# LYL232/Experiment-Distributed-Deep-Learning

Hardware: AMD Instinct MI355X
Metric: device-resident allreduce GiB/s vs bucket size at 1/2/4/8 MI355X (higher is better)
Workload: dtype f32; 1 GPU; C2: local reduce kernel acc += in (per-hop ring reduce), fp32, 256 MiB bucket, 1xMI355X; bucket_bytes=268435456, parallelism=none (1 GPU)

## Files before the change

experiment-distributed-deep-learning_amd/csrc/c_api.cpp:

```cpp
#include <algorithm>
#include <cstdlib>
#include <cstring>
#include <map>
#include <memory>
#include <string>
#include <tuple>
#include <vector>

#include "engine.h"
#include "abi.h"
#include "handler.h"

using namespace ddl;
using namespace ddl::abi;

namespace {

std::shared_ptr<ReadyEvent> ready_event(int memory, void *hip_stream) {
    DDL_REQUIRE(memory == DDL_MEMORY_DEVICE || memory == DDL_MEMORY_HOST, DDL_STATUS_INVALID_ARGUMENT,
                "memory must be DDL_MEMORY_DEVICE (0) or DDL_MEMORY_HOST (1), not " << memory);
    return memory == DDL_MEMORY_HOST ? nullptr : std::make_shared<ReadyEvent>(as_stream(hip_stream));
}

}

extern "C" {

int ddl_version(void) { return 2; }

#ifndef DDL_SRC_HASH
#define DDL_SRC_HASH "unknown"
#endif
const char *ddl_build_info(void) { return "src=" DDL_SRC_HASH " arch=gfx950"; }
const char *ddl_last_error(void) { return last_error(); }
const char *ddl_dtype_name(int dtype) { return dtype_name(dtype); }
size_t ddl_dtype_size(int dtype) { return dtype_size(dtype); }

int ddl_get_unique_id(void *out, size_t len) {
    return guarded([&] {
        DDL_REQUIRE(out && len >= sizeof(ncclUniqueId), DDL_STATUS_INVALID_ARGUMENT,
                    "unique id buffer needs " << sizeof(ncclUniqueId) << " bytes");
        ncclUniqueId id;
        rccl_check(rccl().GetUniqueId(&id), "ncclGetUniqueId");
        std::memcpy(out, &id, sizeof id);
    });
}

int ddl_init(int rank, int size, int device, const void *unique_id, size_t len) {
    return guarded([&] {
        DDL_REQUIRE(size >= 1 && rank >= 0 && rank < size, DDL_STATUS_INVALID_ARGUMENT,
                    "bad rank/size " << rank << "/" << size);
        DDL_REQUIRE(!Registry::get().initialized(), DDL_STATUS_INVALID_ARGUMENT, "already initialized");
        DDL_HIP(hipSetDevice(device));
        ncclComm_t nc = size > 1 ? rccl_init_rank(rank, size, unique_id, len) : nullptr;
        Registry::get().set_world(new_communicator(rank, size, device, nc));
        DDL_LOG(1, "initialized rank " << rank << "/" << size << " on device " << device
                                       << (size > 1 ? std::string(" rccl=") + rccl().path : ""));
    });
}

int ddl_init_single(int device) { return ddl_init(0, 1, device, nullptr, 0); }

int ddl_control_listen(char *endpoint_out, size_t len) {
    return guarded([&] {
        std::string ep = standalone_control()->listen();
        DDL_REQUIRE(endpoint_out && len > ep.size(), DDL_STATUS_INVALID_ARGUMENT, "endpoint buffer too small");
        std::memcpy(endpoint_out, ep.c_str(), ep.size() + 1);
    });
}

int ddl_control_connect(const char *endpoints) {
    return guarded([&] {
        DDL_REQUIRE(endpoints, DDL_STATUS_INVALID_ARGUMENT, "null endpoints");
        auto world = Registry::get().world();
        auto ch = standalone_control();
        ch->connect(world->rank(), world->size(), split_endpoints(endpoints), 120000);
        standalone_control() = std::make_shared<ControlChannel>();
        world->enable_keyed(ch);
    });
}

int ddl_control_stats(long long *string_rounds, long long *cached_rounds) {
    return guarded([&] {
        DDL_REQUIRE(string_rounds && cached_rounds, DDL_STATUS_INVALID_ARGUMENT, "null output");
        ControlChannel *ch = standalone_control().get();
        if (Registry::get().initialized() && Registry::get().world()->control())
            ch = Registry::get().world()->control();
        *string_rounds = ch->string_rounds;
        *cached_rounds = ch->cached_rounds;
    });
}

int ddl_finalize(void) {
    return guarded([&] {
        Registry::get().clear();
        DDL_REQUIRE(wait_deferred_deletions(60000), DDL_STATUS_ERROR_UNKNOWN,
                    "a communicator released by its own handler thread is still being destroyed after 60 s");
        free_retired();
        standalone_control() = std::make_shared<ControlChannel>();
        run_finalize_hooks();
    });
}

int ddl_is_initialized(void) { return Registry::get().initialized() ? 1 : 0; }

int ddl_set_config(const char *key, long long value) {
    return guarded([&] {
        DDL_REQUIRE(key, DDL_STATUS_INVALID_ARGUMENT, "null key");
        std::string k(key);
        Config &c = config();
        if (k == "slice_bytes") c.slice_bytes = value;
        else if (k == "algo") {
            DDL_REQUIRE(value >= kAlgoRing && value <= kAlgoDirectGather, DDL_STATUS_INVALID_ARGUMENT,
                        "algo must be 0 (ring), 1 (direct), 2 (one-shot), 3 (gather-fold) or 4 (direct-gather)");
            c.algo = value;
        } else if (k == "rings") c.rings = value;
        else if (k == "max_slices") c.max_slices = value;
        else if (k == "fusion_threshold_bytes") {
            DDL_REQUIRE(value > 0, DDL_STATUS_INVALID_ARGUMENT, "fusion threshold must be > 0");
            c.fusion_threshold_bytes = value;
        } else if (k == "log_level") c.log_level = value;
        else if (k == "cycle_time_us") c.cycle_time_us = value;
        else if (k == "host_chunk_bytes") {
            DDL_REQUIRE(value >= 4096, DDL_STATUS_INVALID_ARGUMENT, "host_chunk_bytes must be >= 4096");
            c.host_chunk_bytes = value;
        } else if (k == "host_copy_threads") {
            DDL_REQUIRE(value >= 0 && value <= 64, DDL_STATUS_INVALID_ARGUMENT, "host_copy_threads must be in [0, 64]");
            c.host_copy_threads = value;
        } else if (k == "host_zero_copy") c.host_zero_copy = value ? 1 : 0;
        else if (k == "host_numa_bind") c.host_numa_bind = value ? 1 : 0;
        else if (k == "host_register_cache_bytes") {
            DDL_REQUIRE(value >= 0, DDL_STATUS_INVALID_ARGUMENT, "host_register_cache_bytes must be >= 0");
            c.host_register_cache_bytes = value;
            if (value == 0)
                for (auto &comm : Registry::get().all())
                    if (RequestHandler *h = comm->handler_if_created()) h->release_registrations();
        }
        else if (k == "tune") c.tune = value ? 1 : 0;
        else if (k == "fusion_pipeline_bytes") {
            DDL_REQUIRE(value >= 0, DDL_STATUS_INVALID_ARGUMENT, "fusion_pipeline_bytes must be >= 0");
            c.fusion_pipeline_bytes = value;
        } else if (k == "one_rank_shortcut") c.one_rank_shortcut = value ? 1 : 0;
        else if (k == "pipeline_rounds") c.pipeline_rounds = value ? 1 : 0;
        else if (k == "reference_order") c.reference_order = value ? 1 : 0;
        else if (k == "capture_mode") {
            DDL_REQUIRE(value != 1, DDL_STATUS_INVALID_ARGUMENT,
                        "capture_mode 1 (forked streams) was removed in r04: HIP 7.0's hipStreamEndCapture crashes "
                        "on three or more cross-waiting forked streams (DESIGN §9); 2 keeps the overlap");
            DDL_REQUIRE(value == 0 || value == 2, DDL_STATUS_INVALID_ARGUMENT,
                        "capture_mode must be 0 (serial) or 2 (single-stream DAG)");
            c.capture_mode = value;
        } else if (k == "compute_cu_mask") {
            DDL_REQUIRE(value == 0 || value == 2 || value == 4 || value == 8, DDL_STATUS_INVALID_ARGUMENT,
                        "compute_cu_mask must be 0 (all CUs), 2, 4 or 8 (every n-th CU left to RCCL)");
            c.compute_cu_mask = value;
        } else if (k == "queue_isolation") c.queue_isolation = value ? 1 : 0;
        else if (k == "rccl_min_ctas" || k == "rccl_max_ctas") {
            DDL_REQUIRE(value >= 0 && value <= 256, DDL_STATUS_INVALID_ARGUMENT,
                        k << " must be 0 (RCCL's default) or a channel count in [1, 256]");
            (k == "rccl_min_ctas" ? c.rccl_min_ctas : c.rccl_max_ctas) = value;
        } else if (k == "fold_form") {
            DDL_REQUIRE(value >= 0 && value <= 2, DDL_STATUS_INVALID_ARGUMENT,
                        "fold_form must be 0 (auto), 1 (tile form) or 2 (run form)");
            set_fold_form((int)value);
        }
        else fail(DDL_STATUS_INVALID_ARGUMENT, "unknown config key '" + k + "'");
        c.epoch.fetch_add(1);
    });
}

long long ddl_get_config(const char *key) {
    if (!key) return -1;
    std::string k(key);
    Config &c = config();
    if (k == "slice_bytes") return c.slice_bytes;
    if (k == "algo") return c.algo;
    if (k == "rings") return c.rings;
    if (k == "max_slices") return c.max_slices;
    if (k == "fusion_threshold_bytes") return c.fusion_threshold_bytes;
    if (k == "log_level") return c.log_level;
    if (k == "cycle_time_us") return c.cycle_time_us;
    if (k == "host_chunk_bytes") return c.host_chunk_bytes;
    if (k == "tune") return c.tune;
    if (k == "host_copy_threads") return c.host_copy_threads;
    if (k == "host_zero_copy") return c.host_zero_copy;
    if (k == "host_register_cache_bytes") return c.host_register_cache_bytes;
    if (k == "host_numa_bind") return c.host_numa_bind;
    if (k == "host_registered_bytes") return c.host_registered_bytes;
    if (k == "host_register_failures") return c.host_register_failures;
    if (k == "host_register_hits") return c.host_register_hits;
    if (k == "host_unregistered_ranges") return c.host_unregistered_ranges;
    if (k == "host_zero_copy_plans") return c.host_zero_copy_plans;
    if (k == "host_pack_us") return c.host_pack_ns / 1000;
    if (k == "host_wait_us") return c.host_wait_ns / 1000;
    if (k == "host_unpack_us") return c.host_unpack_ns / 1000;
    if (k == "host_check_us") return c.host_check_ns / 1000;
    if (k == "host_plan_us") return c.host_plan_ns / 1000;
    if (k == "host_coll_us") return c.host_coll_ns / 1000;
    if (k == "host_d2h_post_us") return c.host_d2h_post_ns / 1000;
    if (k == "host_unpack_submit_us") return c.host_unpack_submit_ns / 1000;
    if (k == "host_lane_d2h_wait_us") return c.host_lane_d2h_wait_ns / 1000;
    if (k == "host_lane_copy_us") return c.host_lane_copy_ns / 1000;
    if (k == "host_lane_copy_bytes") return c.host_lane_copy_bytes;
    if (k == "host_lane_jobs") return c.host_lane_jobs;
    if (k == "fusion_pipeline_bytes") return c.fusion_pipeline_bytes;
    if (k == "one_rank_shortcut") return c.one_rank_shortcut;
    if (k == "pipeline_rounds") return c.pipeline_rounds;
    if (k == "reference_order") return c.reference_order;
    if (k == "capture_mode") return c.capture_mode;
    if (k == "fold_form") return get_fold_form();
    if (k == "compute_cu_mask") return c.compute_cu_mask;
    if (k == "queue_isolation") return c.queue_isolation;
    if (k == "rccl_min_ctas") return c.rccl_min_ctas;
    if (k == "rccl_max_ctas") return c.rccl_max_ctas;
    return -1;
}

int communicator_rank(ddl_communicator_id id) {
    int r = -1;
    if (guarded([&] { r = Registry::get().find(id)->rank(); }) != DDL_STATUS_OK) return -1;
    return r;
}

int communicator_size(ddl_communicator_id id) {
    int s = -1;
    if (guarded([&] { s = Registry::get().find(id)->size(); }) != DDL_STATUS_OK) return -1;
    return s;
}

ddl_communicator_id world_communicator(void) {
    ddl_communicator_id id = 0;
    if (guarded([&] { id = Registry::get().world()->id(); }) != DDL_STATUS_OK) return 0;
    return id;
}

ddl_communicator_id split_communicator(ddl_communicator_id id, int color, int key) {
    ddl_communicator_id out = 0;
    int st = guarded([&] {
        auto c = Registry::get().find(id)->split(color, key);
        Registry::get().add(c);
        out = c->id();
    });
    return st == DDL_STATUS_OK ? out : 0;
}

void detach_communicator(ddl_communicator_id id) {
    (void)guarded([&] { Registry::get().detach(id); });
}

void py_info(const char *s) { DDL_LOG(1, "[py]: " << (s ? s : "")); }
void py_debug(const char *s) { DDL_LOG(2, "[py]: " << (s ? s : "")); }
void py_error(const char *s) { DDL_LOG(0, "[py]: " << (s ? s : "")); }

int ddl_allreduce(ddl_communicator_id id, const void *send, void *recv, size_t elements, int dtype,
                  int op, void *hip_stream) {
    return guarded([&] { Registry::get().find(id)->allreduce(send, recv, elements, dtype, op, as_stream(hip_stream)); });
}

int ddl_allreduce_batch(ddl_communicator_id id, int count, const void *const *sends, void *const *recvs,
                        const size_t *elements, int dtype, int op, void *hip_stream) {
    return guarded([&] {
        Registry::get().find(id)->allreduce_batch(sends, recvs, elements, count, dtype, op, as_stream(hip_stream));
    });
}

int ddl_broadcast(ddl_communicator_id id, void *buf, size_t elements, int dtype, int root, void *hip_stream) {
    return guarded([&] { Registry::get().find(id)->broadcast(buf, elements, dtype, root, as_stream(hip_stream)); });
}

int ddl_allgatherv(ddl_communicator_id id, const void *send, size_t send_elements, void *recv,
                   const size_t *recv_counts, const size_t *displs, int dtype, void *hip_stream) {
    return guarded([&] {
        auto c = Registry::get().find(id);
        DDL_REQUIRE(recv_counts && displs, DDL_STATUS_INVALID_ARGUMENT, "null counts/displs");
        DDL_REQUIRE(recv_counts[c->rank()] == send_elements, DDL_STATUS_INVALID_ARGUMENT,
                    "send_elements " << send_elements << " != recv_counts[rank] " << recv_counts[c->rank()]);
        c->allgatherv(send, recv, recv_counts, displs, dtype, as_stream(hip_stream));
    });
}

int ddl_allgather(ddl_communicator_id id, const void *send, size_t send_elements, void *recv, size_t recv_elements,
                  int dtype, void *hip_stream) {
    return guarded([&] {
        auto c = Registry::get().find(id);
        DDL_REQUIRE(send_elements == recv_elements, DDL_STATUS_INVALID_ARGUMENT,
                    "send_elements " << send_elements << " != recv_elements " << recv_elements);
        std::vector<size_t> counts(c->size(), recv_elements), displs(c->size());
        for (int q = 0; q < c->size(); ++q) displs[q] = (size_t)q * recv_elements;
        c->allgatherv(send, recv, counts.data(), displs.data(), dtype, as_stream(hip_stream));
    });
}

int ddl_allreduce_host(ddl_communicator_id id, const void *send, void *recv, size_t elements, int dtype, int op) {
    return guarded([&] { Registry::get().find(id)->allreduce_host(send, recv, elements, dtype, op); });
}

int ddl_comm_transport(ddl_communicator_id id, int *kind, int *ranks) {
    return guarded([&] {
        DDL_REQUIRE(kind && ranks, DDL_STATUS_INVALID_ARGUMENT, "null output");
        Registry::get().find(id)->transport(kind, ranks);
    });
}

int ddl_tune_result(ddl_communicator_id id, size_t bucket_bytes, int *chosen, int *count, long long *configs,
                    float *ms, int max_candidates) {
    return guarded([&] {
        export_tune(Registry::get().find(id)->tune_result(bucket_bytes), chosen, count, configs, ms, max_candidates);
    });
}

int ddl_allreduce_submit_mem(ddl_communicator_id id, const char *key, const void *in, void *out, size_t elements,
                             int dtype, int op, int memory, void *hip_stream, ddl_done_fn done, void *user) {
    return guarded([&] {
        DDL_REQUIRE(key, DDL_STATUS_INVALID_ARGUMENT, "null key");
        auto c = Registry::get().find(id);
        DeviceGuard g(c->device());
        Request r;
        r.key = key;
        r.in = in;
        r.out = out;
        r.n = elements;
        r.dtype = dtype;
        r.op = op;
        r.done = done;
        r.user = user;
        r.host = memory == DDL_MEMORY_HOST;
        r.ready = ready_event(memory, hip_stream);
        c->handler().submit(r);
    });
}

int ddl_allreduce_submit(ddl_communicator_id id, const char *key, const void *in, void *out, size_t elements,
                         int dtype, int op, void *hip_stream, ddl_done_fn done, void *user) {
    return ddl_allreduce_submit_mem(id, key, in, out, elements, dtype, op, DDL_MEMORY_DEVICE, hip_stream, done, user);
}

int ddl_broadcast_submit_mem(ddl_communicator_id id, const char *key, const void *in, void *out, size_t elements,
                             int dtype, int root, int memory, void *hip_stream, ddl_done_fn done, void *user) {
    return guarded([&] {
        DDL_REQUIRE(key, DDL_STATUS_INVALID_ARGUMENT, "null key");
        auto c = Registry::get().find(id);
        DeviceGuard g(c->device());
        Request r;
        r.type = kReqBroadcast;
        r.key = key;
        r.in = in;
        r.out = out;
        r.n = elements;
        r.dtype = dtype;
        r.root = root;
        r.done = done;
        r.user = user;
        r.host = memory == DDL_MEMORY_HOST;
        r.ready = ready_event(memory, hip_stream);
        c->handler().submit(r);
    });
}

int ddl_broadcast_submit(ddl_communicator_id id, const char *key, const void *in, void *out, size_t elements,
                         int dtype, int root, void *hip_stream, ddl_done_fn done, void *user) {
    return ddl_broadcast_submit_mem(id, key, in, out, elements, dtype, root, DDL_MEMORY_DEVICE, hip_stream, done,
                                    user);
}

int ddl_allgather_submit_mem(ddl_communicator_id id, const char *key, const void *in, size_t first_dim,
                             size_t row_elements, int dtype, int memory, void *hip_stream, ddl_alloc_fn alloc,
                             ddl_done_fn done, void *user) {
    return guarded([&] {
        DDL_REQUIRE(key, DDL_STATUS_INVALID_ARGUMENT, "null key");
        auto c = Registry::get().find(id);
        DeviceGuard g(c->device());
        Request r;
        r.type = kReqAllgather;
        r.key = key;
        r.in = in;
        r.first_dim = first_dim;
        r.row_elems = row_elements;
        r.n = first_dim * row_elements;
        r.dtype = dtype;
        r.alloc = alloc;
        r.done = done;
        r.user = user;
        r.host = memory == DDL_MEMORY_HOST;
        r.ready = ready_event(memory, hip_stream);
        c->handler().submit(r);
    });
}

int ddl_allgather_submit(ddl_communicator_id id, const char *key, const void *in, size_t first_dim, size_t row_elements,
                         int dtype, void *hip_stream, ddl_alloc_fn alloc, ddl_done_fn done, void *user) {
    return ddl_allgather_submit_mem(id, key, in, first_dim, row_elements, dtype, DDL_MEMORY_DEVICE, hip_stream, alloc,
                                    done, user);
}

int ddl_allreduce_submit_batch_mem(ddl_communicator_id id, int count, const char *const *keys, const void *const *ins,
                                   void *const *outs, const size_t *elements, const int *dtypes, int op, int memory,
                                   void *hip_stream, ddl_done_fn done, void *const *users) {
    return guarded([&] {
        DDL_REQUIRE(count >= 0 && (count == 0 || (keys && ins && outs && elements && dtypes)),
                    DDL_STATUS_INVALID_ARGUMENT, "bad batch arguments");
        if (count == 0) return;
        auto c = Registry::get().find(id);
        DeviceGuard g(c->device());
        auto ready = ready_event(memory, hip_stream);
        std::vector<Request> rs(count);
        for (int i = 0; i < count; ++i) {
            DDL_REQUIRE(keys[i], DDL_STATUS_INVALID_ARGUMENT, "null key " << i);
            rs[i].key = keys[i];
            rs[i].in = ins[i];
            rs[i].out = outs[i];
            rs[i].n = elements[i];
            rs[i].dtype = dtypes[i];
            rs[i].op = op;
            rs[i].done = done;
            rs[i].user = users ? users[i] : nullptr;
            rs[i].host = memory == DDL_MEMORY_HOST;
            rs[i].ready = ready;
        }
        c->handler().submit_batch(rs);
    });
}

int ddl_allreduce_submit_batch(ddl_communicator_id id, int count, const char *const *keys, const void *const *ins,
                               void *const *outs, const size_t *elements, const int *dtypes, int op,
                               void *hip_stream, ddl_done_fn done, void *const *users) {
    return ddl_allreduce_submit_batch_mem(id, count, keys, ins, outs, elements, dtypes, op, DDL_MEMORY_DEVICE,
                                          hip_stream, done, users);
}

int ddl_kernel_timing(ddl_communicator_id id, int on) {
    return guarded([&] {
        auto c = Registry::get().find(id);
        std::lock_guard<std::mutex> g(c->mutex());
        c->executor().set_timing(on != 0);
    });
}

int ddl_kernel_stats(ddl_communicator_id id, long long *launches, double *bytes, double *ms) {
    return guarded([&] {
        DDL_REQUIRE(launches && bytes && ms, DDL_STATUS_INVALID_ARGUMENT, "null output");
        auto c = Registry::get().find(id);
        std::lock_guard<std::mutex> g(c->mutex());
        DeviceGuard dg(c->device());
        KernelStats s = c->executor().collect_stats();
        *launches = s.launches;
        *bytes = s.bytes;
        *ms = s.ms;
    });
}

int ddl_host_unregister(const void *ptr, size_t bytes) {
    return guarded([&] {
        for (auto &comm : Registry::get().all())
            if (RequestHandler *h = comm->handler_if_created()) h->unregister_range(ptr, bytes);
    });
}

int ddl_wait_all(ddl_communicator_id id) {
    return guarded([&] { Registry::get().find(id)->handler().wait_all(); });
}

}
```

experiment-distributed-deep-learning_amd/csrc/common.h:

```cpp
#pragma once

#include <hip/hip_runtime.h>

#include <algorithm>
#include <cstddef>
#include <cstdint>
#include <cstdio>
#include <string>
#include <sstream>
#include <vector>

#include "ddl_amd_testing.h"

namespace ddl {

inline size_t dtype_size(int dt) {
    switch (dt) {
        case DDL_FLOAT: case DDL_INT32: return 4;
        case DDL_DOUBLE: case DDL_INT64: case DDL_UINT64: return 8;
        case DDL_HALF: case DDL_BFLOAT16: return 2;
        default: return 0;
    }
}

inline const char *dtype_name(int dt) {
    switch (dt) {
        case DDL_FLOAT: return "float32";
        case DDL_DOUBLE: return "float64";
        case DDL_INT32: return "int32";
        case DDL_INT64: return "int64";
        case DDL_UINT64: return "uint64";
        case DDL_HALF: return "float16";
        case DDL_BFLOAT16: return "bfloat16";
        default: return "unsupported";
    }
}

void set_error(const std::string &msg);
const char *last_error();

struct Error {
    int status;
    std::string msg;
};

[[noreturn]] inline void fail(int status, const std::string &msg) { throw Error{status, msg}; }

#define DDL_HIP(expr)                                                                       \
    do {                                                                                    \
        hipError_t _e = (expr);                                                             \
        if (_e != hipSuccess) {                                                             \
            std::ostringstream _os;                                                         \
            _os << #expr << " failed: " << hipGetErrorString(_e) << " (" << __FILE__ << ":" \
                << __LINE__ << ")";                                                         \
            ::ddl::fail(DDL_STATUS_HIP_ERROR, _os.str());                                   \
        }                                                                                   \
    } while (0)

#define DDL_REQUIRE(cond, status, msg)                    \
    do {                                                  \
        if (!(cond)) {                                    \
            std::ostringstream _os;                       \
            _os << msg;                                   \
            ::ddl::fail((status), _os.str());             \
        }                                                 \
    } while (0)

int log_level();
void log_line(int level, const std::string &msg);

#define DDL_LOG(level, msg)                                     \
    do {                                                        \
        if (::ddl::log_level() >= (level)) {                    \
            std::ostringstream _os;                             \
            _os << msg;                                         \
            ::ddl::log_line((level), _os.str());                \
        }                                                       \
    } while (0)

#define DDL_TRACE(msg)                                                                          \
    do {                                                                                        \
        if (::ddl::log_level() >= 4) {                                                          \
            std::ostringstream _os;                                                             \
            _os << msg;                                                                         \
            std::fprintf(stderr, "[ddl trace] %s\n", _os.str().c_str());                         \
            std::fflush(stderr);                                                                \
        }                                                                                       \
    } while (0)

constexpr int kMaxSegments = 8;

struct SegTable {
    const void *a[kMaxSegments];
    const void *b[kMaxSegments];
    void *out[kMaxSegments];
    uint64_t n[kMaxSegments];
    int count;
};

constexpr int kMaxInputs = 15;
enum FoldOrder : int {
    kFoldLeft = 0,
    kFoldMpichTree = 1,
    kFoldBinomial = 2,
};
inline int mpich_fold_order(size_t message_bytes, size_t esize, int P) {
    size_t pof2 = 1;
    while (pof2 * 2 <= (size_t)P) pof2 *= 2;
    return message_bytes <= 2048 || message_bytes / esize < pof2 ? kFoldBinomial : kFoldMpichTree;
}
struct SegTableN {
    const void *a;
    const void *b[kMaxInputs];
    void *out;
    uint64_t n;
    int nb;
    int order = kFoldLeft;
};
void launch_sumN(const SegTableN &t, int dtype, hipStream_t stream);
constexpr int kMaxFoldBatch = 8;
struct FoldBatch {
    SegTableN t[kMaxFoldBatch];
    int count;
};
void launch_sumN_batch(const SegTableN *t, int count, int dtype, hipStream_t stream);

enum ReduceVariant : int {
    kNtLoadA = 1,
    kNtLoadB = 2,
    kNtStore = 4,
    kLdsStageB = 8,
    kWtStore = 16,
    kVariantMask = 31,
    kRunForm = 32,
    kRun4 = 64,
};
int default_variant(size_t bytes);
int ring_variant();
void set_fold_form(int form);
void set_testing_fold_variant(int v);
int get_fold_form();

void launch_sum2(const SegTable &t, int dtype, hipStream_t stream, int variant = -1);
int device_cu_count();

inline std::vector<size_t> host_chunk_cuts(size_t total, size_t chunk) {
    std::vector<size_t> cut{0};
    while (cut.back() < total) cut.push_back(cut.back() + std::min(chunk, total - cut.back()));
    return cut;
}

class SegmentCopier {
public:
    SegmentCopier() = default;
    ~SegmentCopier();
    SegmentCopier(const SegmentCopier &) = delete;
    SegmentCopier &operator=(const SegmentCopier &) = delete;
    void run(int dir, void *flat, void *const *segs, const size_t *bytes, int count, hipStream_t stream);
    static size_t flat_bytes(const size_t *bytes, int count);

private:
    struct Slot {
        void *host = nullptr, *dev = nullptr;
        size_t cap = 0;
        void *idx = nullptr;
        size_t idx_cap = 0;
        hipEvent_t ready = nullptr;
    };
    Slot &free_slot_();
    static constexpr size_t kMaxSlots = 64;
    std::vector<Slot> slots_;
    size_t next_ = 0;
};

void retire_device(void *p);
void retire_host(void *p);
void free_retired();
void *thread_scratch(size_t bytes);

enum class QueueClass { kPooled, kHigh, kLow };

}
```

experiment-distributed-deep-learning_amd/csrc/engine.h:

```cpp
#pragma once

#include <atomic>
#include <condition_variable>
#include <functional>
#include <map>
#include <memory>
#include <mutex>
#include <string>
#include <utility>
#include <vector>

#include "control.h"
#include "executor.h"

namespace ddl {

class RequestHandler;

struct Config {
    std::atomic<long long> algo{kAlgoRing};
    std::atomic<long long> slice_bytes{2ll << 20};
    std::atomic<long long> rings{kMaxRings};
    std::atomic<long long> max_slices{8};
    std::atomic<long long> fusion_threshold_bytes{(1ll << 31) - 1};
    std::atomic<long long> log_level{0};
    std::atomic<long long> cycle_time_us{0};
    std::atomic<long long> host_chunk_bytes{32ll << 20};
    std::atomic<long long> host_copy_threads{7};
    std::atomic<long long> host_zero_copy{1};
    std::atomic<long long> host_register_cache_bytes{0};
    std::atomic<long long> host_numa_bind{1};
    std::atomic<long long> host_registered_bytes{0};
    std::atomic<long long> host_register_failures{0};
    std::atomic<long long> host_register_hits{0};
    std::atomic<long long> host_unregistered_ranges{0};
    std::atomic<long long> host_zero_copy_plans{0};
    std::atomic<long long> host_pack_ns{0};
    std::atomic<long long> host_wait_ns{0};
    std::atomic<long long> host_unpack_ns{0};
    std::atomic<long long> host_check_ns{0};
    std::atomic<long long> host_plan_ns{0};
    std::atomic<long long> host_coll_ns{0};
    std::atomic<long long> host_d2h_post_ns{0};
    std::atomic<long long> host_unpack_submit_ns{0};
    std::atomic<long long> host_lane_d2h_wait_ns{0};
    std::atomic<long long> host_lane_copy_ns{0};
    std::atomic<long long> host_lane_copy_bytes{0};
    std::atomic<long long> host_lane_jobs{0};
    std::atomic<long long> tune{1};
    std::atomic<long long> fusion_pipeline_bytes{256ll << 20};
    std::atomic<long long> one_rank_shortcut{1};
    std::atomic<long long> pipeline_rounds{1};
    std::atomic<long long> reference_order{1};
    std::atomic<long long> capture_mode{0};
    std::atomic<long long> compute_cu_mask{0};
    std::atomic<long long> rccl_min_ctas{0};
    std::atomic<long long> rccl_max_ctas{0};
    std::atomic<long long> queue_isolation{0};
    std::atomic<long long> epoch{0};
    uint64_t shared_hash() const;
    RingConfig ring() const {
        RingConfig c;
        c.algo = (int)algo.load();
        c.rings = (int)rings.load();
        c.slice_bytes = (size_t)slice_bytes.load();
        c.max_slices = (int)max_slices.load();
        c.ref_order = reference_order.load() ? 1 : 0;
        return c;
    }
};
Config &config();

struct TuneResult {
    std::vector<RingConfig> candidates;
    std::vector<float> ms;
    int chosen = -1;
};

int size_class(size_t bytes);

TuneResult run_tuning(int P, size_t bytes, hipStream_t stream, const RingConfig &base,
                      const std::function<void(const RingConfig &)> &run,
                      const std::function<void(float *, int)> &agree_max);

class Communicator {
public:
    Communicator(int rank, int size, int device, ncclComm_t nccl, std::shared_ptr<TestHooks> hooks = nullptr,
                 long long tag = 0, std::vector<int> world_ranks = {}, QueueClass qc = QueueClass::kPooled);
    ~Communicator();

    long long id() const { return reinterpret_cast<long long>(this); }
    int rank() const { return rank_; }
    int size() const { return size_; }
    int device() const { return device_; }
    QueueClass queue_class() const { return qclass_; }
    QueueClass keyed_queue_class() const { return keyed_qclass_; }
    ncclComm_t nccl() const { return nccl_; }

    void allreduce(const void *send, void *recv, size_t n, int dtype, int op, hipStream_t stream,
                   size_t order_bytes = 0);
    void allreduce_batch(const void *const *send, void *const *recv, const size_t *n, int count, int dtype, int op,
                         hipStream_t stream);
    void allreduce_host(const void *send, void *recv, size_t n, int dtype, int op);
    void broadcast(void *buf, size_t n, int dtype, int root, hipStream_t stream);
    void allgatherv(const void *send, void *recv, const size_t *counts, const size_t *displs, int dtype,
                    hipStream_t stream);
    std::shared_ptr<Communicator> split(int color, int key, bool keyed = true);

    RingConfig ring_config(size_t n, int dtype, hipStream_t stream);
    TuneResult tune_result(size_t bytes);

    RequestHandler &handler();
    RequestHandler *handler_if_created();
    ControlChannel *control() const { return control_.get(); }
    void enable_keyed(std::shared_ptr<ControlChannel> ch);
    std::shared_ptr<Communicator> keyed_data() const { return keyed_data_; }
    RingExecutor &executor() { return *exec_; }
    std::mutex &mutex() { return mu_; }
    void rccl_allreduce(const void *send, void *recv, size_t n, int dtype, hipStream_t stream);
    void transport(int *kind, int *ranks) const;

    long long round_freeze();
    void round_release(long long at);
    void round_enter(long long at);
    void round_unfreeze();
    void round_abort(int status, const std::string &why);
    long long user_collectives() const;
    std::vector<long long> round_log() const;

    void agree_config(hipStream_t stream);

private:
    class UserCollective;
    std::mutex gate_mu_;
    std::condition_variable gate_cv_;
    long long user_seq_ = 0;
    long long user_done_ = 0;
    bool frozen_ = false;
    int aborted_ = 0;
    std::string abort_msg_;
    long long release_ = 0;
    std::vector<long long> round_log_;
    uint64_t agreed_hash_ = 0;
    uint64_t tuned_hash_ = 0;
    hipStream_t ctl_stream_ = nullptr;
    void agree_max_(float *values, int count, hipStream_t stream);

    int rank_, size_, device_;
    ncclComm_t nccl_;
    std::shared_ptr<TestHooks> hooks_;
    long long tag_ = 0;
    std::vector<int> world_ranks_;
    Transport *cb_ = nullptr;
    std::mutex mu_;
    std::unique_ptr<RingExecutor> exec_;
    std::shared_ptr<ControlChannel> control_;
    std::shared_ptr<Communicator> keyed_data_;
    std::unique_ptr<RequestHandler> handler_;
    std::mutex handler_mu_;
    std::map<int, TuneResult> tuned_;
    TuneResult tune_(size_t n, int dtype, hipStream_t stream, const RingConfig &base);
    hipStream_t h2d_ = nullptr, ring_ = nullptr, d2h_ = nullptr;
    static constexpr int kHostSlots = 4;
    void *slots_[kHostSlots] = {};
    size_t slot_bytes_ = 0;
    void *tune_a_ = nullptr, *tune_b_ = nullptr;
    size_t tune_cap_ = 0;
    QueueClass qclass_ = QueueClass::kPooled, keyed_qclass_ = QueueClass::kPooled;
};

extern thread_local bool t_handler_thread;

struct CommunicatorDeleter {
    void operator()(Communicator *c) const;
};
bool wait_deferred_deletions(long long limit_ms);


template <class... A>
std::shared_ptr<Communicator> new_communicator(A &&...a) {
    return std::shared_ptr<Communicator>(new Communicator(std::forward<A>(a)...), CommunicatorDeleter{});
}

class Registry {
public:
    static Registry &get();
    void add(const std::shared_ptr<Communicator> &c);
    std::shared_ptr<Communicator> find(long long id);
    void detach(long long id);
    std::shared_ptr<Communicator> world();
    std::vector<std::shared_ptr<Communicator>> all();
    void set_world(const std::shared_ptr<Communicator> &c);
    void clear();
    bool initialized();

private:
    std::mutex mu_;
    std::map<long long, std::shared_ptr<Communicator>> comms_;
    std::shared_ptr<Communicator> world_;
};

void add_finalize_hook(void (*fn)());
void run_finalize_hooks();

class DeviceGuard {
public:
    explicit DeviceGuard(int device);
    ~DeviceGuard();

private:
    int prev_ = -1;
};

ncclComm_t rccl_init_rank(int rank, int size, const void *unique_id, size_t len);
ncclComm_t rccl_split(ncclComm_t parent, int color, int key, int *rank, int *size);
void rccl_max_floats(ncclComm_t comm, float *values, int count, hipStream_t stream);
void rccl_allgather_u64(ncclComm_t comm, uint64_t *values, int size, int rank, hipStream_t stream);
void check_config_agreement(int rank, const std::vector<uint64_t> &hashes);

}
```

experiment-distributed-deep-learning_amd/csrc/pack.hip:

```cpp
#include <hip/hip_runtime.h>

#include <algorithm>
#include <cstdlib>
#include <cstring>
#include <mutex>
#include <vector>

#include "common.h"
#include "deptrace.h"

namespace ddl {

namespace {

using u32x4 = unsigned int __attribute__((ext_vector_type(4)));

struct SegDesc {
    uint64_t ptr;
    uint64_t off;
    uint64_t len;
    uint32_t vec;
    uint32_t tile0;
};

__device__ inline void copy_bytes(char *dst, const char *src, uint32_t m) {
    for (uint32_t k = 0; k < m; ++k) dst[k] = src[k];
}

constexpr uint32_t kIdxBlock = 128;

template <bool NARROW>
__global__ void __launch_bounds__(256) k_tile_index(const SegDesc *__restrict__ d, int count, uint64_t tiles,
                                                    const uint32_t *__restrict__ base, void *__restrict__ map) {
    const uint64_t t = (uint64_t)blockIdx.x * 256 + threadIdx.x;
    if (t >= tiles) return;
    int lo = 0, hi = count;
    while (hi - lo > 1) {
        const int mid = (lo + hi) >> 1;
        if (d[mid].tile0 <= t) lo = mid;
        else hi = mid;
    }
    if (NARROW) static_cast<uint8_t *>(map)[t] = (uint8_t)(lo - (int)base[t / kIdxBlock]);
    else static_cast<int *>(map)[t] = lo;
}

template <int DIR, int kIters, int THREADS, bool NARROW>
__global__ void __launch_bounds__(THREADS) k_seg_tiles(char *flat, const SegDesc *__restrict__ d,
                                                       const uint32_t *__restrict__ blk_base,
                                                       const void *__restrict__ map) {
    constexpr uint64_t kTile = (uint64_t)THREADS * 16 * kIters;
    const unsigned tile = blockIdx.x;
    const int seg = NARROW ? (int)(blk_base[tile / kIdxBlock] +
                                   ((static_cast<const uint32_t *>(map)[tile / 4] >> (8 * (tile % 4))) & 0xffu))
                           : static_cast<const int *>(map)[tile];
    const SegDesc sd = d[seg];
    const uint64_t base = (uint64_t)(tile - sd.tile0) * kTile;
    char *fl = flat + sd.off;
    char *tp = reinterpret_cast<char *>(sd.ptr);
    if (!sd.vec) {
        for (uint64_t b = base + threadIdx.x; b < sd.len && b < base + kTile; b += THREADS) {
            if (DIR == 0) fl[b] = tp[b];
            else tp[b] = fl[b];
        }
        return;
    }
    u32x4 v[kIters];
#pragma unroll
    for (int it = 0; it < kIters; ++it) {
        const uint64_t b = base + (uint64_t)it * THREADS * 16 + threadIdx.x * 16;
        if (b + 16 <= sd.len)
            v[it] = __builtin_nontemporal_load(reinterpret_cast<const u32x4 *>((DIR == 0 ? tp : fl) + b));
    }
#pragma unroll
    for (int it = 0; it < kIters; ++it) {
        const uint64_t b = base + (uint64_t)it * THREADS * 16 + threadIdx.x * 16;
        if (b + 16 <= sd.len) {
            __builtin_nontemporal_store(v[it], reinterpret_cast<u32x4 *>((DIR == 0 ? fl : tp) + b));
        } else if (b < sd.len) {
            const uint32_t m = (uint32_t)(sd.len - b);
            if (DIR == 0) copy_bytes(fl + b, tp + b, m);
            else copy_bytes(tp + b, fl + b, m);
        }
    }
}

constexpr uint64_t kSegTile = 1024;
template <int DIR, bool NARROW>
void launch_dir(dim3 g, hipStream_t stream, char *fl, const SegDesc *dd, const uint32_t *db, const void *map) {
    hipLaunchKernelGGL((k_seg_tiles<DIR, 1, 64, NARROW>), g, dim3(64), 0, stream, fl, dd, db, map);
}

void launch_tiles(int dir, bool narrow, dim3 g, hipStream_t stream, char *fl, const SegDesc *dd, const uint32_t *db,
                  const void *map) {
    if (dir == 0) {
        if (narrow) launch_dir<0, true>(g, stream, fl, dd, db, map);
        else launch_dir<0, false>(g, stream, fl, dd, db, map);
    } else {
        if (narrow) launch_dir<1, true>(g, stream, fl, dd, db, map);
        else launch_dir<1, false>(g, stream, fl, dd, db, map);
    }
}

}

SegmentCopier::~SegmentCopier() {
    for (Slot &sl : slots_) {
        if (sl.ready) (void)hipEventSynchronize(sl.ready);
        if (sl.ready) (void)hipEventDestroy(sl.ready);
        if (sl.host) (void)hipHostFree(sl.host);
        if (sl.dev) (void)hipFree(sl.dev);
        if (sl.idx) (void)hipFree(sl.idx);
    }
}

SegmentCopier::Slot &SegmentCopier::free_slot_() {
    for (size_t k = 0; k < slots_.size(); ++k) {
        Slot &sl = slots_[(next_ + k) % slots_.size()];
        if (!sl.ready) continue;
        const hipError_t q = hipEventQuery(sl.ready);
        if (q == hipErrorNotReady) continue;
        DDL_HIP(q);
        next_ = (next_ + k + 1) % slots_.size();
        return sl;
    }
    if (slots_.size() < kMaxSlots) {
        slots_.emplace_back();
        Slot &sl = slots_.back();
        DDL_HIP(hipEventCreateWithFlags(&sl.ready, hipEventDisableTiming));
        next_ = 0;
        return sl;
    }
    Slot &sl = slots_[next_];
    next_ = (next_ + 1) % slots_.size();
    DDL_HIP(hipEventSynchronize(sl.ready));
    return sl;
}

size_t SegmentCopier::flat_bytes(const size_t *bytes, int count) {
    size_t off = 0;
    for (int i = 0; i < count; ++i) off += (bytes[i] + 255) & ~size_t(255);
    return off;
}

void SegmentCopier::run(int dir, void *flat, void *const *segs, const size_t *bytes, int count,
                        hipStream_t stream) {
    if (count <= 0) return;
    DDL_REQUIRE(flat && segs && bytes, DDL_STATUS_INVALID_ARGUMENT, "null pack arguments");
    Slot &sl = free_slot_();
    const uint64_t seg_tile = kSegTile;
    uint64_t tiles = 0;
    for (int i = 0; i < count; ++i) tiles += (bytes[i] + seg_tile - 1) / seg_tile;
    DDL_REQUIRE(tiles < (1ull << 31), DDL_STATUS_INVALID_ARGUMENT, "fusion buffer too large");
    const uint64_t nblk = (tiles + kIdxBlock - 1) / kIdxBlock;
    const size_t table = (size_t)count * sizeof(SegDesc);
    const size_t need = table + nblk * sizeof(uint32_t);
    if (need > sl.cap) {
        retire_host(sl.host);
        retire_device(sl.dev);
        sl.host = sl.dev = nullptr;
        sl.cap = need + need / 2;
        DDL_HIP(hipHostMalloc(&sl.host, sl.cap, hipHostMallocDefault));
        DDL_HIP(hipMalloc(&sl.dev, sl.cap));
    }
    SegDesc *t = static_cast<SegDesc *>(sl.host);
    uint32_t *bases = reinterpret_cast<uint32_t *>(static_cast<char *>(sl.host) + table);
    uint64_t off = 0, tl = 0;
    for (int i = 0; i < count; ++i) {
        DDL_REQUIRE(bytes[i] == 0 || segs[i], DDL_STATUS_INVALID_ARGUMENT, "null segment " << i);
        t[i].ptr = reinterpret_cast<uint64_t>(segs[i]);
        t[i].off = off;
        t[i].len = bytes[i];
        t[i].vec = (reinterpret_cast<uintptr_t>(segs[i]) & 15u) == 0;
        t[i].tile0 = (uint32_t)tl;
        off += (bytes[i] + 255) & ~uint64_t(255);
        tl += (bytes[i] + seg_tile - 1) / seg_tile;
    }
    if (off == 0) return;
    bool narrow = true;
    for (uint64_t b = 0, s0 = 0, s1 = 0; b < nblk; ++b) {
        const uint64_t first = b * kIdxBlock, last = std::min(tiles, first + kIdxBlock) - 1;
        while (s0 + 1 < (uint64_t)count && t[s0 + 1].tile0 <= first) ++s0;
        if (s1 < s0) s1 = s0;
        while (s1 + 1 < (uint64_t)count && t[s1 + 1].tile0 <= last) ++s1;
        bases[b] = (uint32_t)s0;
        if (s1 - s0 > 255) narrow = false;
    }
    DDL_HIP(hipMemcpyAsync(sl.dev, sl.host, need, hipMemcpyHostToDevice, stream));
    char *fl = static_cast<char *>(flat);
    const SegDesc *dd = static_cast<const SegDesc *>(sl.dev);
    const uint32_t *db = reinterpret_cast<const uint32_t *>(static_cast<char *>(sl.dev) + table);
    if (tiles > 0) {
        const size_t ib = narrow ? (tiles + 3) & ~uint64_t(3) : tiles * sizeof(int);
        if (ib > sl.idx_cap) {
            retire_device(sl.idx);
            sl.idx = nullptr;
            sl.idx_cap = ib + ib / 2;
            DDL_HIP(hipMalloc(&sl.idx, sl.idx_cap));
        }
        const dim3 ig((unsigned)((tiles + 255) / 256)), g((unsigned)tiles);
        if (narrow) hipLaunchKernelGGL(k_tile_index<true>, ig, dim3(256), 0, stream, dd, count, (uint64_t)tiles, db, sl.idx);
        else hipLaunchKernelGGL(k_tile_index<false>, ig, dim3(256), 0, stream, dd, count, (uint64_t)tiles, db, sl.idx);
        launch_tiles(dir, narrow, g, stream, fl, dd, db, sl.idx);
    }
    DDL_HIP(hipGetLastError());
    DDL_HIP(hipEventRecord(sl.ready, stream));
    if (dep::on()) {
        std::vector<dep::Access> acc;
        acc.push_back(dir == 0 ? dep::wr(flat, off) : dep::rd(flat, off));
        for (int i = 0; i < count; ++i)
            if (bytes[i]) acc.push_back(dir == 0 ? dep::rd(segs[i], bytes[i]) : dep::wr(segs[i], bytes[i]));
        dep::op(stream, dir == 0 ? "pack" : "unpack", std::move(acc));
    }
}

}
```

experiment-distributed-deep-learning_amd/ddl/torch/config.py:

```python
import contextlib

from ddl.torch.cpp_backend import CPPBackend, check

KEYS = ('algo', 'slice_bytes', 'rings', 'max_slices', 'fusion_threshold_bytes', 'log_level', 'cycle_time_us',
        'host_chunk_bytes', 'host_copy_threads', 'host_zero_copy', 'tune', 'fusion_pipeline_bytes', 'one_rank_shortcut',
        'pipeline_rounds', 'reference_order', 'host_register_cache_bytes', 'capture_mode',
        'fold_form', 'compute_cu_mask', 'host_numa_bind', 'rccl_min_ctas', 'rccl_max_ctas', 'queue_isolation')
SHARED = ('algo', 'slice_bytes', 'rings', 'max_slices', 'fusion_threshold_bytes', 'tune', 'fusion_pipeline_bytes',
          'reference_order', 'host_chunk_bytes', 'rccl_min_ctas', 'rccl_max_ctas')


def set(key: str, value: int) -> None:
    check(CPPBackend.c_api().ddl_set_config(key.encode(), int(value)), f'ddl_set_config({key})')


def get(key: str) -> int:
    return int(CPPBackend.c_api().ddl_get_config(key.encode()))


def snapshot() -> dict:
    return {k: get(k) for k in KEYS}


@contextlib.contextmanager
def override(**values):
    old = {k: get(k) for k in values}
    try:
        for k, v in values.items():
            set(k, v)
        yield
    finally:
        for k, v in old.items():
            set(k, v)
```

Measured before the change: 2071 GiB/s.

## Cache device-side pack segment tables and tile indices across calls

```diff
diff --git a/experiment-distributed-deep-learning_amd/csrc/c_api.cpp b/experiment-distributed-deep-learning_amd/csrc/c_api.cpp
--- a/experiment-distributed-deep-learning_amd/csrc/c_api.cpp
+++ b/experiment-distributed-deep-learning_amd/csrc/c_api.cpp
@@ -141,7 +141,10 @@
             DDL_REQUIRE(value >= 0, DDL_STATUS_INVALID_ARGUMENT, "fusion_pipeline_bytes must be >= 0");
             c.fusion_pipeline_bytes = value;
         } else if (k == "one_rank_shortcut") c.one_rank_shortcut = value ? 1 : 0;
-        else if (k == "pipeline_rounds") c.pipeline_rounds = value ? 1 : 0;
+        else if (k == "pack_table_cache_entries" || k == "pack_table_cache_max_bytes") {
+            DDL_REQUIRE(value >= 0, DDL_STATUS_INVALID_ARGUMENT, k << " must be >= 0");
+            (k == "pack_table_cache_entries" ? c.pack_table_cache_entries : c.pack_table_cache_max_bytes) = value;
+        } else if (k == "pipeline_rounds") c.pipeline_rounds = value ? 1 : 0;
         else if (k == "reference_order") c.reference_order = value ? 1 : 0;
         else if (k == "capture_mode") {
             DDL_REQUIRE(value != 1, DDL_STATUS_INVALID_ARGUMENT,
@@ -205,6 +208,11 @@
     if (k == "host_lane_jobs") return c.host_lane_jobs;
     if (k == "fusion_pipeline_bytes") return c.fusion_pipeline_bytes;
     if (k == "one_rank_shortcut") return c.one_rank_shortcut;
+    if (k == "pack_table_cache_entries") return c.pack_table_cache_entries;
+    if (k == "pack_table_cache_max_bytes") return c.pack_table_cache_max_bytes;
+    if (k == "pack_table_cache_hits") return c.pack_table_cache_hits;
+    if (k == "pack_table_cache_misses") return c.pack_table_cache_misses;
+    if (k == "pack_table_cache_bytes") return c.pack_table_cache_bytes;
     if (k == "pipeline_rounds") return c.pipeline_rounds;
     if (k == "reference_order") return c.reference_order;
     if (k == "capture_mode") return c.capture_mode;
diff --git a/experiment-distributed-deep-learning_amd/csrc/common.h b/experiment-distributed-deep-learning_amd/csrc/common.h
--- a/experiment-distributed-deep-learning_amd/csrc/common.h
+++ b/experiment-distributed-deep-learning_amd/csrc/common.h
@@ -162,7 +162,7 @@
 private:
     struct Slot {
         void *host = nullptr, *dev = nullptr;
-        size_t cap = 0;
+        size_t host_cap = 0, cap = 0;
         void *idx = nullptr;
         size_t idx_cap = 0;
         hipEvent_t ready = nullptr;
@@ -171,6 +171,32 @@
     static constexpr size_t kMaxSlots = 64;
     std::vector<Slot> slots_;
     size_t next_ = 0;
+
+    struct Built {
+        uint64_t tiles = 0, flat = 0;
+        size_t table = 0, need = 0, idx_bytes = 0;
+        bool narrow = true;
+    };
+    Built build_(Slot &sl, void *const *segs, const size_t *bytes, int count);
+    struct Entry {
+        uint64_t hash = 0;
+        std::vector<uint64_t> ptrs, lens;
+        void *dev = nullptr, *idx = nullptr;
+        size_t cap = 0, idx_cap = 0;
+        Built b;
+        hipEvent_t used = nullptr;
+        hipStream_t stream = nullptr;
+        uint64_t tick = 0;
+    };
+    int lru_idle_();
+    Entry take_(int k);
+    void retire_(Entry &e);
+    void trim_(size_t entries, size_t bytes);
+    Entry *find_(uint64_t hash, void *const *segs, const size_t *bytes, int count);
+    Entry *admit_(size_t entries, size_t max_bytes, size_t need, size_t idx_need);
+    std::vector<Entry> cache_;
+    size_t cache_bytes_ = 0;
+    uint64_t tick_ = 0;
 };
 
 void retire_device(void *p);
diff --git a/experiment-distributed-deep-learning_amd/csrc/engine.h b/experiment-distributed-deep-learning_amd/csrc/engine.h
--- a/experiment-distributed-deep-learning_amd/csrc/engine.h
+++ b/experiment-distributed-deep-learning_amd/csrc/engine.h
@@ -50,6 +50,11 @@
     std::atomic<long long> tune{1};
     std::atomic<long long> fusion_pipeline_bytes{256ll << 20};
     std::atomic<long long> one_rank_shortcut{1};
+    std::atomic<long long> pack_table_cache_entries{64};
+    std::atomic<long long> pack_table_cache_max_bytes{64ll << 20};
+    std::atomic<long long> pack_table_cache_hits{0};
+    std::atomic<long long> pack_table_cache_misses{0};
+    std::atomic<long long> pack_table_cache_bytes{0};
     std::atomic<long long> pipeline_rounds{1};
     std::atomic<long long> reference_order{1};
     std::atomic<long long> capture_mode{0};
diff --git a/experiment-distributed-deep-learning_amd/csrc/pack.hip b/experiment-distributed-deep-learning_amd/csrc/pack.hip
--- a/experiment-distributed-deep-learning_amd/csrc/pack.hip
+++ b/experiment-distributed-deep-learning_amd/csrc/pack.hip
@@ -8,6 +8,7 @@
 
 #include "common.h"
 #include "deptrace.h"
+#include "engine.h"
 
 namespace ddl {
 
@@ -111,6 +112,13 @@
         if (sl.dev) (void)hipFree(sl.dev);
         if (sl.idx) (void)hipFree(sl.idx);
     }
+    for (Entry &e : cache_) {
+        if (e.used) (void)hipEventSynchronize(e.used);
+        if (e.used) (void)hipEventDestroy(e.used);
+        if (e.dev) (void)hipFree(e.dev);
+        if (e.idx) (void)hipFree(e.idx);
+    }
+    config().pack_table_cache_bytes -= (long long)cache_bytes_;
 }
 
 SegmentCopier::Slot &SegmentCopier::free_slot_() {
@@ -142,11 +150,34 @@
     return off;
 }
 
-void SegmentCopier::run(int dir, void *flat, void *const *segs, const size_t *bytes, int count,
-                        hipStream_t stream) {
-    if (count <= 0) return;
-    DDL_REQUIRE(flat && segs && bytes, DDL_STATUS_INVALID_ARGUMENT, "null pack arguments");
-    Slot &sl = free_slot_();
+namespace {
+
+void grow_device(void *&p, size_t &cap, size_t need) {
+    if (need <= cap) return;
+    retire_device(p);
+    p = nullptr;
+    cap = 0;
+    DDL_HIP(hipMalloc(&p, need + need / 2));
+    cap = need + need / 2;
+}
+
+uint64_t list_hash(void *const *segs, const size_t *bytes, int count) {
+    uint64_t h = 0x9e3779b97f4a7c15ull ^ (uint64_t)count;
+    auto mix = [&h](uint64_t v) {
+        h ^= v;
+        h *= 0xff51afd7ed558ccdull;
+        h ^= h >> 32;
+    };
+    for (int i = 0; i < count; ++i) {
+        mix(reinterpret_cast<uint64_t>(segs[i]));
+        mix((uint64_t)bytes[i]);
+    }
+    return h;
+}
+
+}
+
+SegmentCopier::Built SegmentCopier::build_(Slot &sl, void *const *segs, const size_t *bytes, int count) {
     const uint64_t seg_tile = kSegTile;
     uint64_t tiles = 0;
     for (int i = 0; i < count; ++i) tiles += (bytes[i] + seg_tile - 1) / seg_tile;
@@ -154,13 +185,12 @@
     const uint64_t nblk = (tiles + kIdxBlock - 1) / kIdxBlock;
     const size_t table = (size_t)count * sizeof(SegDesc);
     const size_t need = table + nblk * sizeof(uint32_t);
-    if (need > sl.cap) {
+    if (need > sl.host_cap) {
         retire_host(sl.host);
-        retire_device(sl.dev);
-        sl.host = sl.dev = nullptr;
-        sl.cap = need + need / 2;
-        DDL_HIP(hipHostMalloc(&sl.host, sl.cap, hipHostMallocDefault));
-        DDL_HIP(hipMalloc(&sl.dev, sl.cap));
+        sl.host = nullptr;
+        sl.host_cap = 0;
+        DDL_HIP(hipHostMalloc(&sl.host, need + need / 2, hipHostMallocDefault));
+        sl.host_cap = need + need / 2;
     }
     SegDesc *t = static_cast<SegDesc *>(sl.host);
     uint32_t *bases = reinterpret_cast<uint32_t *>(static_cast<char *>(sl.host) + table);
@@ -175,7 +205,12 @@
         off += (bytes[i] + 255) & ~uint64_t(255);
         tl += (bytes[i] + seg_tile - 1) / seg_tile;
     }
-    if (off == 0) return;
+    Built out;
+    out.tiles = tiles;
+    out.flat = off;
+    out.table = table;
+    out.need = need;
+    if (off == 0) return out;
     bool narrow = true;
     for (uint64_t b = 0, s0 = 0, s1 = 0; b < nblk; ++b) {
         const uint64_t first = b * kIdxBlock, last = std::min(tiles, first + kIdxBlock) - 1;
@@ -185,25 +220,179 @@
         bases[b] = (uint32_t)s0;
         if (s1 - s0 > 255) narrow = false;
     }
-    DDL_HIP(hipMemcpyAsync(sl.dev, sl.host, need, hipMemcpyHostToDevice, stream));
-    char *fl = static_cast<char *>(flat);
-    const SegDesc *dd = static_cast<const SegDesc *>(sl.dev);
-    const uint32_t *db = reinterpret_cast<const uint32_t *>(static_cast<char *>(sl.dev) + table);
-    if (tiles > 0) {
-        const size_t ib = narrow ? (tiles + 3) & ~uint64_t(3) : tiles * sizeof(int);
-        if (ib > sl.idx_cap) {
-            retire_device(sl.idx);
-            sl.idx = nullptr;
-            sl.idx_cap = ib + ib / 2;
-            DDL_HIP(hipMalloc(&sl.idx, sl.idx_cap));
-        }
-        const dim3 ig((unsigned)((tiles + 255) / 256)), g((unsigned)tiles);
-        if (narrow) hipLaunchKernelGGL(k_tile_index<true>, ig, dim3(256), 0, stream, dd, count, (uint64_t)tiles, db, sl.idx);
-        else hipLaunchKernelGGL(k_tile_index<false>, ig, dim3(256), 0, stream, dd, count, (uint64_t)tiles, db, sl.idx);
-        launch_tiles(dir, narrow, g, stream, fl, dd, db, sl.idx);
-    }
+    out.narrow = narrow;
+    out.idx_bytes = narrow ? (tiles + 3) & ~uint64_t(3) : tiles * sizeof(int);
+    return out;
+}
+
+int SegmentCopier::lru_idle_() {
+    std::vector<int> order(cache_.size());
+    for (size_t k = 0; k < order.size(); ++k) order[k] = (int)k;
+    std::sort(order.begin(), order.end(), [&](int a, int b) { return cache_[a].tick < cache_[b].tick; });
+    for (int k : order) {
+        const hipError_t q = hipEventQuery(cache_[k].used);
+        if (q == hipErrorNotReady) continue;
+        DDL_HIP(q);
+        return k;
+    }
+    return -1;
+}
+
+SegmentCopier::Entry SegmentCopier::take_(int k) {
+    Entry e = std::move(cache_[k]);
+    cache_[k] = std::move(cache_.back());
+    cache_.pop_back();
+    cache_bytes_ -= e.cap + e.idx_cap;
+    config().pack_table_cache_bytes -= (long long)(e.cap + e.idx_cap);
+    return e;
+}
+
+void SegmentCopier::retire_(Entry &e) {
+    retire_device(e.dev);
+    retire_device(e.idx);
+    e.dev = e.idx = nullptr;
+    e.cap = e.idx_cap = 0;
+}
+
+void SegmentCopier::trim_(size_t entries, size_t bytes) {
+    while (cache_.size() > entries || cache_bytes_ > bytes) {
+        const int k = lru_idle_();
+        if (k < 0) return;
+        Entry e = take_(k);
+        retire_(e);
+        (void)hipEventDestroy(e.used);
+    }
+}
+
+SegmentCopier::Entry *SegmentCopier::find_(uint64_t hash, void *const *segs, const size_t *bytes, int count) {
+    static_assert(sizeof(void *) == sizeof(uint64_t) && sizeof(size_t) == sizeof(uint64_t), "64-bit key words");
+    for (Entry &e : cache_) {
+        if (e.hash != hash || e.ptrs.size() != (size_t)count) continue;
+        if (std::memcmp(e.ptrs.data(), segs, (size_t)count * sizeof(uint64_t)) != 0) continue;
+        if (std::memcmp(e.lens.data(), bytes, (size_t)count * sizeof(uint64_t)) != 0) continue;
+        return &e;
+    }
+    return nullptr;
+}
+
+SegmentCopier::Entry *SegmentCopier::admit_(size_t entries, size_t max_bytes, size_t need, size_t idx_need) {
+    if (need + idx_need > max_bytes) return nullptr;
+    Entry e;
+    while (cache_.size() >= entries || cache_bytes_ + need + idx_need > max_bytes) {
+        const int k = lru_idle_();
+        if (k < 0) break;
+        retire_(e);
+        if (e.used) (void)hipEventDestroy(e.used);
+        e = take_(k);
+    }
+    const bool room = cache_.size() < entries && cache_bytes_ + need + idx_need <= max_bytes;
+    if (!room || cache_bytes_ + std::max(e.cap, need) + std::max(e.idx_cap, idx_need) > max_bytes) retire_(e);
+    if (!room) {
+        if (e.used) (void)hipEventDestroy(e.used);
+        return nullptr;
+    }
+    if (!e.used) DDL_HIP(hipEventCreateWithFlags(&e.used, hipEventDisableTiming));
+    e.ptrs.clear();
+    e.lens.clear();
+    cache_.push_back(std::move(e));
+    Entry &n = cache_.back();
+    if (n.cap < need) {
+        retire_device(n.dev);
+        n.dev = nullptr;
+        n.cap = 0;
+        DDL_HIP(hipMalloc(&n.dev, need));
+        n.cap = need;
+    }
+    if (n.idx_cap < idx_need) {
+        retire_device(n.idx);
+        n.idx = nullptr;
+        n.idx_cap = 0;
+        DDL_HIP(hipMalloc(&n.idx, idx_need));
+        n.idx_cap = idx_need;
+    }
+    cache_bytes_ += n.cap + n.idx_cap;
+    config().pack_table_cache_bytes += (long long)(n.cap + n.idx_cap);
+    return &n;
+}
+
+void SegmentCopier::run(int dir, void *flat, void *const *segs, const size_t *bytes, int count,
+                        hipStream_t stream) {
+    if (count <= 0) return;
+    DDL_REQUIRE(flat && segs && bytes, DDL_STATUS_INVALID_ARGUMENT, "null pack arguments");
+    Config &cfg = config();
+    const size_t max_entries = (size_t)std::max(0ll, cfg.pack_table_cache_entries.load());
+    const size_t max_bytes = (size_t)std::max(0ll, cfg.pack_table_cache_max_bytes.load());
+    bool cached = false;
+    if (max_entries > 0 || !cache_.empty()) {
+        hipStreamCaptureStatus cs = hipStreamCaptureStatusNone;
+        if (hipStreamIsCapturing(stream, &cs) != hipSuccess) {
+            (void)hipGetLastError();
+            cs = hipStreamCaptureStatusActive;
+        }
+        if (cs == hipStreamCaptureStatusNone) {
+            trim_(max_entries, max_entries ? max_bytes : 0);
+            cached = max_entries > 0;
+        }
+    }
+    Entry *e = nullptr;
+    uint64_t hash = 0;
+    if (cached) {
+        hash = list_hash(segs, bytes, count);
+        e = find_(hash, segs, bytes, count);
+    }
+    Built b;
+    Slot *sl = nullptr;
+    if (e) {
+        ++cfg.pack_table_cache_hits;
+        b = e->b;
+        if (stream != e->stream) {
+            const hipError_t q = hipEventQuery(e->used);
+            if (q == hipErrorNotReady) DDL_HIP(hipStreamWaitEvent(stream, e->used, 0));
+            else DDL_HIP(q);
+        }
+    } else {
+        sl = &free_slot_();
+        b = build_(*sl, segs, bytes, count);
+        if (b.flat == 0) return;
+        if (cached) {
+            ++cfg.pack_table_cache_misses;
+            e = admit_(max_entries, max_bytes, b.need, b.idx_bytes);
+        }
+        if (!e) {
+            grow_device(sl->dev, sl->cap, b.need);
+            grow_device(sl->idx, sl->idx_cap, b.idx_bytes);
+        }
+        void *dev = e ? e->dev : sl->dev, *idx = e ? e->idx : sl->idx;
+        DDL_HIP(hipMemcpyAsync(dev, sl->host, b.need, hipMemcpyHostToDevice, stream));
+        const SegDesc *dd = static_cast<const SegDesc *>(dev);
+        const uint32_t *db = reinterpret_cast<const uint32_t *>(static_cast<char *>(dev) + b.table);
+        const dim3 ig((unsigned)((b.tiles + 255) / 256));
+        if (b.narrow) hipLaunchKernelGGL(k_tile_index<true>, ig, dim3(256), 0, stream, dd, count, (uint64_t)b.tiles, db, idx);
+        else hipLaunchKernelGGL(k_tile_index<false>, ig, dim3(256), 0, stream, dd, count, (uint64_t)b.tiles, db, idx);
+        if (e) {
+            DDL_HIP(hipGetLastError());
+            DDL_HIP(hipEventRecord(sl->ready, stream));
+        }
+    }
+    void *dev = e ? e->dev : sl->dev;
+    launch_tiles(dir, b.narrow, dim3((unsigned)b.tiles), stream, static_cast<char *>(flat),
+                 static_cast<const SegDesc *>(dev),
+                 reinterpret_cast<const uint32_t *>(static_cast<char *>(dev) + b.table), e ? e->idx : sl->idx);
     DDL_HIP(hipGetLastError());
-    DDL_HIP(hipEventRecord(sl.ready, stream));
+    DDL_HIP(hipEventRecord(e ? e->used : sl->ready, stream));
+    if (e) {
+        if (e->ptrs.empty()) {
+            e->hash = hash;
+            e->ptrs.resize((size_t)count);
+            e->lens.resize((size_t)count);
+            std::memcpy(e->ptrs.data(), segs, (size_t)count * sizeof(uint64_t));
+            std::memcpy(e->lens.data(), bytes, (size_t)count * sizeof(uint64_t));
+            e->b = b;
+        }
+        e->stream = stream;
+        e->tick = ++tick_;
+    }
+    const uint64_t off = b.flat;
     if (dep::on()) {
         std::vector<dep::Access> acc;
         acc.push_back(dir == 0 ? dep::wr(flat, off) : dep::rd(flat, off));
diff --git a/experiment-distributed-deep-learning_amd/ddl/torch/config.py b/experiment-distributed-deep-learning_amd/ddl/torch/config.py
--- a/experiment-distributed-deep-learning_amd/ddl/torch/config.py
+++ b/experiment-distributed-deep-learning_amd/ddl/torch/config.py
@@ -5,7 +5,8 @@
 KEYS = ('algo', 'slice_bytes', 'rings', 'max_slices', 'fusion_threshold_bytes', 'log_level', 'cycle_time_us',
         'host_chunk_bytes', 'host_copy_threads', 'host_zero_copy', 'tune', 'fusion_pipeline_bytes', 'one_rank_shortcut',
         'pipeline_rounds', 'reference_order', 'host_register_cache_bytes', 'capture_mode',
-        'fold_form', 'compute_cu_mask', 'host_numa_bind', 'rccl_min_ctas', 'rccl_max_ctas', 'queue_isolation')
+        'fold_form', 'compute_cu_mask', 'host_numa_bind', 'rccl_min_ctas', 'rccl_max_ctas', 'queue_isolation',
+        'pack_table_cache_entries', 'pack_table_cache_max_bytes')
 SHARED = ('algo', 'slice_bytes', 'rings', 'max_slices', 'fusion_threshold_bytes', 'tune', 'fusion_pipeline_bytes',
           'reference_order', 'host_chunk_bytes', 'rccl_min_ctas', 'rccl_max_ctas')
 
```

Result: no change. 2071 GiB/s (median of 3 runs) (+0.0%).
